# bwa-mem2/bwa-mem2

Hardware: NVIDIA H100
Metric: paired 151bp reads/s (seed+chain+extend hot path) (higher is better)
Workload: dtype int64/int16

## Files before the change

### bwa-mem2_b200/capi.py

```python
from __future__ import annotations
import ctypes as C, os
import numpy as np

_HERE = os.path.dirname(os.path.abspath(__file__))
LIB_PATH = os.path.join(_HERE, "libbm2b200.so")

PAIR_DT = np.dtype([("idr", "<i4"), ("idq", "<i4"), ("id", "<i4"), ("len1", "<i4"), ("len2", "<i4"), ("h0", "<i4"),
                    ("seqid", "<i4"), ("regid", "<i4"), ("score", "<i4"), ("tle", "<i4"), ("gtle", "<i4"),
                    ("qle", "<i4"), ("gscore", "<i4"), ("max_off", "<i4")])
SMEM_DT = np.dtype([("rid", "<u4"), ("m", "<u4"), ("n", "<u4"), ("_pad", "<u4"), ("k", "<i8"), ("l", "<i8"), ("s", "<i8")])
SEED_DT = np.dtype([("rbeg", "<i8"), ("qbeg", "<i4"), ("len", "<i4"), ("score", "<i4"), ("chain", "<i4")])
CHAIN_DT = np.dtype([("pos", "<i8"), ("seqid", "<i4"), ("rid", "<i4"), ("n_seeds", "<i4"), ("seed_off", "<i4"),
                     ("w", "<i4"), ("kept", "<i4"), ("first", "<i4"), ("is_alt", "<i4"), ("frac_rep", "<f4"), ("_pad", "<i4")])
REG_DT = np.dtype([("rb", "<i8"), ("re", "<i8"), ("qb", "<i4"), ("qe", "<i4"), ("rid", "<i4"), ("_p0", "<i4"), ("c", "<u8"),
                   ("score", "<i4"), ("truesc", "<i4"), ("sub", "<i4"), ("alt_sc", "<i4"), ("csub", "<i4"), ("sub_n", "<i4"),
                   ("w", "<i4"), ("seedcov", "<i4"), ("secondary", "<i4"), ("secondary_all", "<i4"), ("seedlen0", "<i4"),
                   ("n_comp_is_alt", "<i4"), ("frac_rep", "<f4"), ("_p1", "<i4"), ("hash", "<u8"), ("flg", "<i4"), ("_p2", "<i4")])


class MemOpt(C.Structure):
    _fields_ = [("a", C.c_int), ("b", C.c_int), ("o_del", C.c_int), ("e_del", C.c_int), ("o_ins", C.c_int), ("e_ins", C.c_int),
                ("pen_unpaired", C.c_int), ("pen_clip5", C.c_int), ("pen_clip3", C.c_int), ("w", C.c_int), ("zdrop", C.c_int),
                ("max_mem_intv", C.c_uint64), ("T", C.c_int), ("flag", C.c_int), ("min_seed_len", C.c_int),
                ("min_chain_weight", C.c_int), ("max_chain_extend", C.c_int), ("split_factor", C.c_float),
# ... 949 lines not shown

    def seed_chain_extend_resident(self, codes, offsets, d_codes_ptr, d_offsets_ptr, copy_out=False, return_arrays=False):
        rb, keep = self._batch(codes, offsets)
        res = RegResult()
        lib().bm2_seed_chain_extend_resident.argtypes = [C.c_void_p, C.c_void_p, C.c_void_p, C.c_void_p, C.c_int, C.c_void_p]
        self._check(lib().bm2_seed_chain_extend_resident(self._ctx, C.byref(rb), d_codes_ptr, d_offsets_ptr, int(copy_out), C.byref(res)),
                    "bm2_seed_chain_extend_resident")
        if not return_arrays:
            return res.n
        n = res.n
        regs = np.ctypeslib.as_array(C.cast(res.regs, C.POINTER(C.c_uint8)), shape=(n * REG_DT.itemsize,)).view(REG_DT).copy() if n else np.zeros(0, REG_DT)
        off = np.ctypeslib.as_array(C.cast(res.read_off, C.POINTER(C.c_int64)), shape=(rb.n_reads + 1,)).copy()
        return regs, off

    def counters(self):
        v = (C.c_ulonglong * 7)()
        lib().bm2_last_counters.argtypes = [C.c_void_p, C.c_void_p, C.c_int]
        lib().bm2_last_counters(self._ctx, v, 7)
        return dict(n_ext=v[0], n_lf=v[1], cells=v[2], retry_left=v[3], retry_right=v[4], jobs_skipped=v[5], reads_done_wave1=v[6])

    def stage_ms(self):
        names = C.POINTER(C.c_char_p)(); ms = C.POINTER(C.c_float)(); n = C.c_int()
        lib().bm2_last_stage_ms(self._ctx, C.byref(names), C.byref(ms), C.byref(n))
        return {names[i].decode(): ms[i] for i in range(n.value)}
```

### bwa-mem2_b200/csrc/bm2_ctx.h

```cpp
#pragma once
#include <cuda_runtime.h>
#include <string>
#include <type_traits>
#include <vector>
#include <mutex>
#include "bm2_b200.h"

struct DevBuf  { void *p = nullptr; size_t cap = 0; };
struct HostBuf { void *p = nullptr; size_t cap = 0; };

struct DevIndex {
    int64_t N = 0, l_pac = 0, sentinel = 0;
    int64_t count[5] = {0, 0, 0, 0, 0};
    const bm2_cp_occ *cp_occ = nullptr;
    int occ_layout = 0;
    const int8_t *sa_ms = nullptr;
    const uint32_t *sa_ls = nullptr;
    const uint8_t *ref = nullptr;
    int32_t n_seqs = 0;
    const int64_t *ann_off = nullptr;
    const int32_t *ann_len = nullptr;
    const int32_t *ann_alt = nullptr;
    bool loaded = false;
};

struct bm2_ctx {
    int device = 0, n_sm = 132;
    int fq_n_reads = 0, fq_n_bufs = 0;
    cudaStream_t stream = nullptr, own_stream = nullptr, side_stream = nullptr;
    cudaEvent_t ev_fork = nullptr, ev_join = nullptr;
    bm2_mem_opt_t opt;
    std::string err;
    DevIndex idx;
    std::vector<void *> idx_allocs;
    DevBuf io_pairs, io_ref, io_qer, bsw_jobs, bsw_outs, bsw_scratch;
    DevBuf pipe_d[39];
    HostBuf pipe_h[5];
    std::vector<cudaEvent_t> events;
    std::vector<const char *> stage_names;
    std::vector<float> stage_ms;
    unsigned long long last_n_ext = 0, last_n_lf = 0, last_cells = 0, last_n_retry[2] = {0, 0};
    unsigned long long last_jobs_skipped = 0, last_walk_done = 0;
    int n_lanes = 4, lane_min_reads = 16384;
    std::vector<bm2_ctx *> lanes;
    bm2_ctx *parent = nullptr;
    std::mutex tok_smem, tok_bsw;
    cudaEvent_t ev_entry = nullptr;
    DevBuf cigar_d[14];
    HostBuf cigar_h[3];
    DevBuf ksw_d[6];
    DevBuf fq_d[38];
    HostBuf fq_h[25];
    DevBuf sam_d[24];
    HostBuf sam_h[5];
    int sam_staged = -1;
    cudaEvent_t sam_ev[5] = {nullptr, nullptr, nullptr, nullptr, nullptr};
    double sam_ms[4] = {0, 0, 0, 0};
// ... 120 lines not shown
```

### bwa-mem2_b200/csrc/fm_device.cuh

```cuda
#pragma once
#include "hd.h"
#include "bm2_b200.h"

struct FmIndexView {
    const bm2_cp_occ *cp_occ;
    const int8_t *sa_ms;
    const uint32_t *sa_ls;
    int64_t count[5];
    int64_t sentinel;
    int layout = 0;
    const uint8_t *text = nullptr;
    int64_t text_len = 0;
};

#if defined(__CUDA_ARCH__)
BM2_D void fm_ld256(const void *p, uint64_t &a, uint64_t &b, uint64_t &c, uint64_t &d) {
    asm volatile("ld.global.nc.v2.u64 {%0,%1}, [%4];\n\t"
                 "ld.global.nc.v2.u64 {%2,%3}, [%4+16];" : "=l"(a), "=l"(b), "=l"(c), "=l"(d) : "l"(p));
}
#endif

struct FmIv { int64_t k, l, s; };

BM2_HD int64_t fm_count(const FmIndexView &fm, int a) {
    return a == 0 ? fm.count[0] : a == 1 ? fm.count[1] : a == 2 ? fm.count[2] : a == 3 ? fm.count[3] : fm.count[4];
}

// ... 62 lines not shown

BM2_HD int64_t fm_sa_of_row(const FmIndexView &fm, int64_t r, int *lf_steps, int64_t at_sentinel = 0) {
    int64_t steps = 0;
    while (r & 7) {
        const bm2_cp_occ *e = fm.cp_occ + (r >> 6);
        const int y = 63 - (int) (r & 63);
#if defined(__CUDA_ARCH__)
        const ulonglong2 *p = reinterpret_cast<const ulonglong2 *>(e);
        ulonglong2 c01 = __ldg(p), c23 = __ldg(p + 1), b01 = __ldg(p + 2), b23 = __ldg(p + 3);
        if (fm.layout) { const ulonglong2 t = c23; c23 = b01; b01 = t; }
        uint64_t cnt[4] = {c01.x, c01.y, c23.x, c23.y}, bits[4] = {b01.x, b01.y, b23.x, b23.y};
#else
        uint64_t cnt[4], bits[4];
        for (int b = 0; b < 4; ++b) { cnt[b] = (uint64_t) e->cp_count[b]; bits[b] = e->one_hot_bwt_str[b]; }
#endif
        int b = ((bits[0] >> y) & 1) ? 0 : ((bits[1] >> y) & 1) ? 1 : ((bits[2] >> y) & 1) ? 2 : ((bits[3] >> y) & 1) ? 3 : 4;
        if (b == 4) { if (lf_steps) *lf_steps += (int) steps; return at_sentinel; }
        const int yy = (int) (r & 63);
        const uint64_t mask = yy ? ~0ULL << (64 - yy) : 0ULL;
        uint64_t cb = b == 0 ? cnt[0] : b == 1 ? cnt[1] : b == 2 ? cnt[2] : cnt[3];
        uint64_t bb = b == 0 ? bits[0] : b == 1 ? bits[1] : b == 2 ? bits[2] : bits[3];
        r = fm_count(fm, b) + (int64_t) cb + BM2_POPC64(bb & mask);
        ++steps;
    }
    if (lf_steps) *lf_steps += (int) steps;
#if defined(__CUDA_ARCH__)
    int64_t sa = ((int64_t) __ldg(fm.sa_ms + (r >> 3)) << 32) + (int64_t) __ldg(fm.sa_ls + (r >> 3));
#else
    int64_t sa = ((int64_t) fm.sa_ms[r >> 3] << 32) + (int64_t) fm.sa_ls[r >> 3];
#endif
    return sa + steps;
}

BM2_HD int64_t fm_text_pos_of_row(const FmIndexView &fm, int64_t r) { return fm_sa_of_row(fm, r, nullptr, -1); }

struct FmPrev { int64_t k, l, s; int32_t m, n; };

struct SmemParams {
    int min_seed_len;
    int split_len;
    int split_width;
    int max_mem_intv;
};

struct QPlain {
    const uint8_t *p;
    BM2_HD int operator()(int j) const { return p[j]; }
};

// ... 56 lines not shown
                if (a > 3) { if (single) return; x = next_x; continue; }
                cur.m = x; cur.n = x; cur.k = fm_count(fm, a); cur.l = fm_count(fm, 3 - a); cur.s = fm_count(fm, a + 1) - cur.k;
                top = cap; j = x + 1; searching = true; tpos = -1;
            }
            bool stop = j >= len;
            if (!stop) { next_x = j + 1; const int a = q(j); if (a > 3) stop = true; else { base = 3 - a; need = true; } }
            if (stop) {
                if (cur.s >= min_intv) scratch[--top] = cur;
                sink(x, min_intv, scratch + top, cap - top);
                if (single) return;
                x = next_x; searching = false;
            }
        }
        BM2_SYNCWARP();
        FmIv r;
        if (fm.text && cur.s == 1 && tpos == -1) tpos = len - j >= 16 ? fm_text_pos_of_row(fm, cur.k) : -2;
        if (fm.text && cur.s == 1 && tpos >= 0) {
            const int64_t tp = tpos + (j - x);
            r.s = (tp < fm.text_len && (int) fm.text[tp] == 3 - base) ? 1 : 0;
            r.l = cur.k; r.k = cur.l;
        } else {
            if (tpos == -1 && fm.text && cur.s == 1) tpos = -2;
            FmIv req; req.k = cur.l; req.l = cur.k; req.s = cur.s;
            r = fm_backward_ext(fm, req, base);
        }
        ++n_ext;
        if (r.s != cur.s) scratch[--top] = cur;
        if (r.s < min_intv) {
            next_x = j;
            if (cur.s >= min_intv) scratch[--top] = cur;
            sink(x, min_intv, scratch + top, cap - top);
            if (single) return;
            x = next_x; searching = false;
        } else { cur.k = r.l; cur.l = r.k; cur.s = r.s; cur.n = j; ++j; }
    }
}

template <class Q, class Emit>
BM2_HD void fm_backward(const FmIndexView &fm, const Q &q, int x, int min_intv, int min_seed_len, FmPrev *pv, int num_prev, Emit &emit,
                        unsigned &n_ext)
{
    int j = x - 1, p = 0, num_curr = 0, curr_s = -1;
    bool first_phase = true;
    for (;;) {
        bool done = false;
        for (;;) {
            if (num_prev == 0 || j < 0) { done = true; break; }
            if (p == 0 && num_curr == 0 && first_phase && q(j) > 3) { done = true; break; }
            if (p < num_prev) break;
            num_prev = num_curr;
            if (num_curr == 0) { done = true; break; }
            --j; p = 0; num_curr = 0; curr_s = -1; first_phase = true;
        }
        if (done) break;
        BM2_SYNCWARP();
        const FmPrev old = pv[p];
        FmIv req; req.k = old.k; req.l = old.l; req.s = old.s;
        const FmIv r = fm_backward_ext(fm, req, q(j));
        ++n_ext;
        if (first_phase && r.s < min_intv && old.n - old.m + 1 >= min_seed_len) {
            emit(old.m, old.n, old.k, old.l, old.s);
            first_phase = false;
        } else if (r.s >= min_intv && r.s != curr_s) {
            curr_s = (int) r.s;
            FmPrev t; t.k = r.k; t.l = r.l; t.s = r.s; t.m = j; t.n = old.n;
            pv[num_curr++] = t;
            first_phase = false;
        }
        ++p;
    }
    if (num_prev != 0) {
        const FmPrev &s0 = pv[0];
        if (s0.n - s0.m + 1 >= min_seed_len) emit(s0.m, s0.n, s0.k, s0.l, s0.s);
    }
}

template <class Q, class Emit>
BM2_HD void fm_backward_rows(const FmIndexView &fm, const Q &q, int x, int min_intv, int min_seed_len, FmPrev *pv, int num_prev,
                             Emit &emit, unsigned &n_ext)
{
    for (int j = x - 1; j >= 0 && num_prev > 0; --j) {
        const int a = q(j);
        if (a > 3) break;
#ifdef BM2_TRACE_BWD_ROW
        BM2_TRACE_BWD_ROW(num_prev);
#endif
        int b = num_prev;
        const FmPrev first = pv[0];
        for (int p = 0; p < num_prev; ++p) {
            FmIv req; req.k = pv[p].k; req.l = pv[p].l; req.s = pv[p].s;
            const FmIv r = fm_backward_ext(fm, req, a);
            ++n_ext;
            pv[p].k = r.k; pv[p].l = r.l; pv[p].s = r.s;
            if (r.s >= min_intv && b == num_prev) b = p;
        }
        if (b > 0 && first.n - first.m + 1 >= min_seed_len) emit(first.m, first.n, first.k, first.l, first.s);
        int num_curr = 0;
        int64_t last_s = -1;
        for (int p = b; p < num_prev; ++p) {
            if (pv[p].s != last_s) { last_s = pv[p].s; FmPrev t = pv[p]; t.m = j; pv[num_curr++] = t; }
        }
        num_prev = num_curr;
    }
    if (num_prev != 0) {
        const FmPrev &s0 = pv[0];
        if (s0.n - s0.m + 1 >= min_seed_len) emit(s0.m, s0.n, s0.k, s0.l, s0.s);
    }
}
```

### bwa-mem2_b200/csrc/pipeline.cu

```cuda
#include "bm2_common.cuh"
#include "bm2_ctx.h"
#include "fm_device.cuh"
#include "chain_device.cuh"
#include "ext_device.cuh"
#include <cub/device/device_radix_sort.cuh>
#include <cub/device/device_scan.cuh>
#include <vector>
#include <algorithm>
#include <mutex>
#include <thread>
#include <string>
#include <cstring>
#include <cstdlib>
#include <cmath>

static_assert(sizeof(ExtJobRec) == sizeof(BswJob), "ExtJobRec must alias BswJob");

int bsw_launch_with_scratch(bm2_ctx *ctx_for_error, cudaStream_t stream, const BswJob *d_jobs, BswOut *d_out, int n,
                            const uint8_t *d_tbase, const uint8_t *d_qbase, const BswParams &prm,
                            unsigned long long *d_cells, void *scratch, size_t scratch_bytes, int wide_possible);

__global__ void occ_relayout_kernel(ulonglong2 *tab, size_t n_entries) {
    const size_t i = (size_t) blockIdx.x * blockDim.x + threadIdx.x;
    if (i >= n_entries) return;
    ulonglong2 *e = tab + i * 4;
    const ulonglong2 c23 = e[1], b01 = e[2];
    e[1] = b01; e[2] = c23;
}

int bm2_upload_index(bm2_ctx *ctx, const bm2_index_desc *idx, int resident) {
    bm2_ctx *ctx_for_error = ctx;
    auto up = [&](const void *src, size_t bytes, const void **dst, bool big) -> int {
        if (big && resident) { *dst = src; return 0; }
        void *p = nullptr;
        BM2_CUDA_OK(cudaMalloc(&p, bytes ? bytes : 1));
        ctx->idx_allocs.push_back(p);
        if (bytes) BM2_CUDA_OK(cudaMemcpy(p, src, bytes, cudaMemcpyHostToDevice));
        *dst = p;
        return 0;
    };
    DevIndex &d = ctx->idx;
    d.N = idx->reference_seq_len; d.l_pac = idx->l_pac; d.sentinel = idx->sentinel_index;
// ... 1 lines not shown
    d.n_seqs = idx->n_seqs;
    size_t n_occ = (size_t) (d.N >> 6) + 1, n_sa = (size_t) (d.N >> 3) + 1;
    if (up(idx->cp_occ, n_occ * sizeof(bm2_cp_occ), (const void **) &d.cp_occ, true)) return 1;
    {
        const char *e = getenv("BM2_OCC_LAYOUT");
        d.occ_layout = (e && e[0] == '0') ? 0 : 1;
        if (d.occ_layout) {
            occ_relayout_kernel<<<(unsigned) ((n_occ + 255) / 256), 256>>>((ulonglong2 *) d.cp_occ, n_occ);
            BM2_CUDA_OK(cudaGetLastError());
            BM2_CUDA_OK(cudaDeviceSynchronize());
        }
    }
    if (up(idx->sa_ms_byte, n_sa, (const void **) &d.sa_ms, true)) return 1;
    if (up(idx->sa_ls_word, n_sa * 4, (const void **) &d.sa_ls, true)) return 1;
    if (up(idx->ref_string, (size_t) d.l_pac * 2, (const void **) &d.ref, true)) return 1;
    if (up(idx->ann_offset, (size_t) d.n_seqs * 8, (const void **) &d.ann_off, false)) return 1;
    if (up(idx->ann_len, (size_t) d.n_seqs * 4, (const void **) &d.ann_len, false)) return 1;
    std::vector<int32_t> zeros;
    const int32_t *alt = idx->ann_is_alt;
    if (!alt) { zeros.assign(d.n_seqs, 0); alt = zeros.data(); }
    if (up(alt, (size_t) d.n_seqs * 4, (const void **) &d.ann_alt, false)) return 1;
    d.loaded = true;
    return 0;
}

void bm2_free_index(bm2_ctx *ctx) {
    for (void *p : ctx->idx_allocs) cudaFree(p);
    ctx->idx_allocs.clear();
    ctx->idx.loaded = false;
}

struct Counters {
    unsigned long long n_smem, n_ext, n_lf, n_retry, cells;
    unsigned long long n_pool, n_task, n_task1, n_rtask;
    unsigned long long n_sel[2], n_walk_done;
};

struct SearchTask { int32_t read, x, min_intv, n; int64_t off; };
struct ReseedTask { int32_t read, x, min_intv; };


struct QShared4 {
    unsigned base, stride;
    __device__ __forceinline__ int operator()(int j) const {
        uint32_t w; asm volatile("ld.shared.u32 %0, [%1];" : "=r"(w) : "r"(base + (unsigned) (j >> 3) * stride));
        return (int) ((w >> ((j & 7) * 4)) & 0xFu);
    }
};

struct PoolSink {
// ... 70 lines not shown
        if (rtasks && n + 1 - m >= split_len && s <= split_width) {
            unsigned long long t = atomicAdd(&cnt->n_rtask, 1ULL);
            if (t < rtask_cap) { ReseedTask r; r.read = (int32_t) rid; r.x = (n + 1 + m) >> 1; r.min_intv = (int32_t) (s + 1); rtasks[t] = r; }
        }
    }
};

#define BWD_G 8
#define BWD_CAP 32
__global__ void __launch_bounds__(128, 8)
smem_bwd_kernel(FmIndexView fm, SmemParams sp, const uint8_t *__restrict__ codes, const int64_t *__restrict__ offs, int round,
                const SearchTask *__restrict__ tasks, unsigned long long task_cap, FmPrev *pool, unsigned long long pool_cap,
                bm2_smem *out, unsigned long long cap, ReseedTask *rtasks, unsigned long long rtask_cap, Counters *cnt)
{
    __shared__ FmPrev shl[128 / BWD_G][BWD_CAP];
    const int lane = threadIdx.x & 31, gl = lane & (BWD_G - 1), gw = lane / BWD_G;
    const unsigned gmask = ((1u << BWD_G) - 1u) << (gw * BWD_G);
    const int grp = (blockIdx.x * blockDim.x + threadIdx.x) / BWD_G, ngrp = gridDim.x * blockDim.x / BWD_G;
    const unsigned long long t0 = round ? cnt->n_task1 : 0ULL;
    const unsigned long long t1 = cnt->n_task < task_cap ? cnt->n_task : task_cap;
    unsigned n_ext = 0;
    for (unsigned long long t = t0 + grp; t < t1; t += ngrp) {
        const SearchTask k = tasks[t];
        if ((unsigned long long) k.off + k.n > pool_cap) continue;
        SmemAppend emit = { out, cap, cnt, (uint32_t) k.read, round ? nullptr : rtasks, rtask_cap, sp.split_len, sp.split_width };
        const uint8_t *q = codes + offs[k.read];
        FmPrev *lst = pool + k.off;
        int num_prev = k.n;
        if (num_prev <= BWD_CAP) {
            FmPrev *sl = shl[threadIdx.x / BWD_G];
            for (int p = gl; p < num_prev; p += BWD_G) sl[p] = lst[p];
            lst = sl;
        }
        __syncwarp(gmask);
        for (int j = k.x - 1; j >= 0 && num_prev > 0; --j) {
            const int a = q[j];
            if (a > 3) break;
            const FmPrev first = lst[0];
            __syncwarp(gmask);
            int b = num_prev;
            for (int p = gl; p < num_prev; p += BWD_G) {
                FmIv req; req.k = lst[p].k; req.l = lst[p].l; req.s = lst[p].s;
                const FmIv r = fm_backward_ext(fm, req, a);
                ++n_ext;
                lst[p].k = r.k; lst[p].l = r.l; lst[p].s = r.s;
                if (r.s >= k.min_intv && p < b) b = p;
            }
#pragma unroll
            for (int d = BWD_G / 2; d > 0; d >>= 1) b = min(b, __shfl_xor_sync(gmask, b, d));
            __syncwarp(gmask);
            if (gl == 0 && b > 0 && first.n - first.m + 1 >= sp.min_seed_len) emit(first.m, first.n, first.k, first.l, first.s);
            int num_curr = 0;
            for (int base = b; base < num_prev; base += BWD_G) {
                const int p = base + gl;
                bool keep = false;
                FmPrev e;
                if (p < num_prev) { e = lst[p]; keep = (p == b) || (lst[p - 1].s != e.s); }
                const unsigned km = __ballot_sync(gmask, keep) >> (gw * BWD_G);
                __syncwarp(gmask);
                if (keep) { e.m = j; lst[num_curr + __popc(km & ((1u << gl) - 1u))] = e; }
                num_curr += __popc(km);
                __syncwarp(gmask);
            }
            num_prev = num_curr;
        }
        if (gl == 0 && num_prev != 0) {
            const FmPrev s0 = lst[0];
            if (s0.n - s0.m + 1 >= sp.min_seed_len) emit(s0.m, s0.n, s0.k, s0.l, s0.s);
        }
        __syncwarp(gmask);
    }
    n_ext = __reduce_add_sync(0xffffffffu, n_ext);
    if (lane == 0 && n_ext) atomicAdd(&cnt->n_ext, (unsigned long long) n_ext);
}

__global__ void mark_task1_kernel(Counters *cnt) { if (threadIdx.x == 0 && blockIdx.x == 0) cnt->n_task1 = cnt->n_task; }

template <bool USE_SMEM>
__global__ void __launch_bounds__(128, 12)
smem_pass3_kernel(FmIndexView fm, SmemParams sp, const uint8_t *__restrict__ codes, const int64_t *__restrict__ offs, int n_reads,
                  bm2_smem *out, unsigned long long cap, Counters *cnt)
{
    extern __shared__ uint32_t qsh[];
    const int tid = blockIdx.x * blockDim.x + threadIdx.x, nthr = gridDim.x * blockDim.x;
    unsigned n_ext = 0;
    for (int r = tid; r < n_reads; r += nthr) {
        const int64_t o = offs[r];
        const int len = (int) (offs[r + 1] - o);
// ... 5 lines not shown
        } else {
            QPlain q = { codes + o };
            fm_smem_pass3(fm, q, len, sp, emit, n_ext);
        }
    }
    if (n_ext) atomicAdd(&cnt->n_ext, (unsigned long long) n_ext);
}

__global__ void smem_keys_kernel(const bm2_smem *sm, int64_t n, uint64_t *keys, uint32_t *vals) {
    int64_t i = (int64_t) blockIdx.x * blockDim.x + threadIdx.x;
    if (i >= n) return;
    keys[i] = (uint64_t) sm[i].rid << 32 | (uint64_t) (sm[i].m & 0xFFFFu) << 16 | (uint64_t) (sm[i].n & 0xFFFFu);
    vals[i] = (uint32_t) i;
}

__global__ void smem_gather_kernel(const bm2_smem *in, const uint32_t *perm, int64_t n, int max_occ, bm2_smem *out, int64_t *slot_cnt) {
    int64_t i = (int64_t) blockIdx.x * blockDim.x + threadIdx.x;
    if (i >= n) return;
    bm2_smem x = in[perm[i]];
    out[i] = x;
    slot_cnt[i] = x.s < max_occ ? x.s : max_occ;
}

__global__ void read_smem_off_kernel(const uint64_t *keys_sorted, int64_t n_smem, int n_reads, int64_t *read_smem_off) {
    int r = blockIdx.x * blockDim.x + threadIdx.x;
    if (r > n_reads) return;
    const uint64_t key = (uint64_t) r << 32;
    int64_t lo = 0, hi = n_smem;
    while (lo < hi) { int64_t mid = (lo + hi) >> 1; if (keys_sorted[mid] < key) lo = mid + 1; else hi = mid; }
    read_smem_off[r] = lo;
}

__global__ void slot_head_kernel(const int64_t *__restrict__ slot_off, int64_t n_smem, int32_t *owner) {
    int64_t i = (int64_t) blockIdx.x * blockDim.x + threadIdx.x;
    if (i >= n_smem) return;
    if (slot_off[i + 1] > slot_off[i]) owner[slot_off[i]] = (int32_t) i;
}

__global__ void __launch_bounds__(256)
sa_kernel(FmIndexView fm, const bm2_smem *__restrict__ sm, const int64_t *__restrict__ slot_off, const int32_t *__restrict__ owner,
          int64_t n_slots, int max_occ, int64_t *sa, Counters *cnt)
{
    int64_t t = (int64_t) blockIdx.x * blockDim.x + threadIdx.x;
    int lf = 0;
    if (t < n_slots) {
        const int32_t o = owner[t];
        const bm2_smem x = sm[o];
        const int64_t step = x.s > max_occ ? x.s / max_occ : 1;
        sa[t] = fm_sa_of_row(fm, x.k + (t - slot_off[o]) * step, &lf);
    }
    lf = __reduce_add_sync(0xffffffffu, lf);
    if ((threadIdx.x & 31) == 0 && lf) atomicAdd(&cnt->n_lf, (unsigned long long) lf);
}

struct ChainBufs {
    WSeed *wseed; WChain *wchain; int32_t *ord, *srt, *kv; int64_t *ordpos; FltRec *flt;
    bm2_chain *fin_chain; bm2_seed *fin_seed;
    int32_t *n_chain, *n_seed, *n_left, *n_right;
};

__global__ void __launch_bounds__(128)
chain_kernel(ContigView cv, ChainParams cp, const bm2_smem *__restrict__ sm, const int64_t *__restrict__ read_smem_off,
             const int64_t *__restrict__ slot_off, const int64_t *__restrict__ sa, const int64_t *__restrict__ offs, int n_reads,
             const int32_t *__restrict__ perm, ChainBufs b, SwParams sw, const uint8_t *__restrict__ ref, const uint8_t *__restrict__ codes,
// ... 529 lines not shown
        for (int r = 0; r < n; ++r) {
            const int64_t l = rb->offsets[r + 1] - rb->offsets[r];
            if (l < 0 || l > 32767) { bm2_set_error(ctx, "read length out of range (0..32767)"); return 1; }
            if (l > max_len) max_len = (int) l;
            if (l != memo_l) {
                const double min_l = ctx->opt.min_chain_weight ? 1.1f * ctx->opt.min_chain_weight : 5.5f * log((double) (l > 0 ? l : 1));
                memo_l = l; memo_hsp = -1;
                if (l > 0 && !(min_l > 0.05f * l)) memo_hsp = (int) (ctx->opt.a * min_l + .499);
            }
            if (memo_hsp >= 0 && !any_flt) { any_flt = true; min_hsp_host.assign((size_t) n, -1); }
            if (any_flt) min_hsp_host[r] = memo_hsp;
        }
    }
    bs.max_len = max_len;
    Params pv = make_params(ctx);
    if (upto != UPTO_SMEM && env_int("BM2_SMEM_TEXT", 1, 0, 1)) { pv.fm.text = ctx->idx.ref; pv.fm.text_len = 2 * ctx->idx.l_pac; }
    Stages sg = { ctx, ctx->events, ctx->stage_names };
    if (sg.mark("h2d")) return 1;

    if (ctx->ensure(ctx->pipe_d[B_CNT], sizeof(Counters))) return 1;
    const uint8_t *d_codes = ext_codes; const int64_t *d_offs = ext_offs;
    if (!ext_codes) {
        if (ctx->ensure(ctx->pipe_d[B_CODES], (size_t) total + 16)) return 1;
        BM2_CUDA_OK(cudaMemcpyAsync(ctx->pipe_d[B_CODES].p, rb->codes, (size_t) total, cudaMemcpyHostToDevice, st));
        d_codes = P<uint8_t>(ctx, B_CODES);
    }
    if (!ext_offs) {
        if (ctx->ensure(ctx->pipe_d[B_OFFS], (size_t) (n + 1) * 8)) return 1;
        BM2_CUDA_OK(cudaMemcpyAsync(ctx->pipe_d[B_OFFS].p, rb->offsets, (size_t) (n + 1) * 8, cudaMemcpyHostToDevice, st));
        d_offs = P<int64_t>(ctx, B_OFFS);
    }
// ... 49 lines not shown
        smem_fwd2_kernel<<<blocks_a, 128, 0, st>>>(pv.fm, d_codes, d_offs, stripe, P<FmPrev>(ctx, B_PREV), d_rt, rtask_cap, d_pool, pool_cap, d_tasks, task_cap, d_cnt);
        smem_bwd_kernel<<<blocks_b, 128, 0, st>>>(pv.fm, pv.sp, d_codes, d_offs, 1, d_tasks, task_cap, d_pool, pool_cap, d_raw, cap, d_rt, rtask_cap, d_cnt);
        BM2_CUDA_OK(cudaStreamWaitEvent(st, ctx->ev_join, 0));
        BM2_CUDA_OK(cudaMemcpyAsync(&h_cnt, d_cnt, sizeof(Counters), cudaMemcpyDeviceToHost, st));
        BM2_CUDA_OK(cudaStreamSynchronize(st));
        if (h_cnt.n_smem <= cap && h_cnt.n_pool <= pool_cap && h_cnt.n_task <= task_cap && h_cnt.n_rtask <= rtask_cap) break;
        if (attempt == 2) { bm2_set_error(ctx, "SMEM stage buffers overflow"); return 1; }
        if (h_cnt.n_smem > cap) cap = h_cnt.n_smem * 2 + 1024;
        if (h_cnt.n_pool > pool_cap) pool_cap = h_cnt.n_pool * 2 + 65536;
        if (h_cnt.n_task > task_cap) task_cap = h_cnt.n_task * 2 + 4096;
        if (h_cnt.n_rtask > rtask_cap) rtask_cap = h_cnt.n_rtask * 2 + 4096;
    }
    tok_smem.release();
    const int64_t n_smem = (int64_t) h_cnt.n_smem;
    bs.n_smem = n_smem;
    ctx->last_n_ext = h_cnt.n_ext;

    if (sg.mark("sort")) return 1;
    const int64_t ns1 = n_smem > 0 ? n_smem : 1;
    if (ctx->ensure(ctx->pipe_d[B_KEYS_IN], ns1 * 8) || ctx->ensure(ctx->pipe_d[B_KEYS_OUT], ns1 * 8) || ctx->ensure(ctx->pipe_d[B_VALS_IN], ns1 * 4) ||
        ctx->ensure(ctx->pipe_d[B_VALS_OUT], ns1 * 4) || ctx->ensure(ctx->pipe_d[B_SMEM], (ns1 + 1) * sizeof(bm2_smem)) ||
        ctx->ensure(ctx->pipe_d[B_SLOT_CNT], (ns1 + 1) * 8) || ctx->ensure(ctx->pipe_d[B_SLOT_OFF], (ns1 + 2) * 8) ||
        ctx->ensure(ctx->pipe_d[B_READ_SMEM_OFF], (size_t) (n + 2) * 8)) return 1;
    if (n_smem > 0) {
        const int gb = (int) ((n_smem + 255) / 256);
        smem_keys_kernel<<<gb, 256, 0, st>>>(P<bm2_smem>(ctx, B_SMEM_RAW), n_smem, P<uint64_t>(ctx, B_KEYS_IN), P<uint32_t>(ctx, B_VALS_IN));
        size_t cub_bytes = 0;
        cub::DeviceRadixSort::SortPairs(nullptr, cub_bytes, P<uint64_t>(ctx, B_KEYS_IN), P<uint64_t>(ctx, B_KEYS_OUT), P<uint32_t>(ctx, B_VALS_IN),
                                        P<uint32_t>(ctx, B_VALS_OUT), (int) n_smem);
        if (ctx->ensure(ctx->pipe_d[B_CUB], cub_bytes)) return 1;
        BM2_CUDA_OK(cub::DeviceRadixSort::SortPairs(ctx->pipe_d[B_CUB].p, cub_bytes, P<uint64_t>(ctx, B_KEYS_IN), P<uint64_t>(ctx, B_KEYS_OUT),
                                                    P<uint32_t>(ctx, B_VALS_IN), P<uint32_t>(ctx, B_VALS_OUT), (int) n_smem, 0, 64, st));
        BM2_CUDA_OK(cudaMemsetAsync(P<int64_t>(ctx, B_SLOT_CNT) + n_smem, 0, 8, st));
        smem_gather_kernel<<<gb, 256, 0, st>>>(P<bm2_smem>(ctx, B_SMEM_RAW), P<uint32_t>(ctx, B_VALS_OUT), n_smem, ctx->opt.max_occ,
                                               P<bm2_smem>(ctx, B_SMEM), P<int64_t>(ctx, B_SLOT_CNT));
    } else {
        BM2_CUDA_OK(cudaMemsetAsync(P<int64_t>(ctx, B_SLOT_CNT), 0, 8, st));
    }
    read_smem_off_kernel<<<(n + 1 + 255) / 256, 256, 0, st>>>(P<uint64_t>(ctx, B_KEYS_OUT), n_smem, n, P<int64_t>(ctx, B_READ_SMEM_OFF));
    if (scan64(ctx, P<int64_t>(ctx, B_SLOT_CNT), P<int64_t>(ctx, B_SLOT_OFF), n_smem)) return 1;
    if (upto == UPTO_SMEM) { if (sg.mark("end")) return 1; BM2_CUDA_OK(cudaStreamSynchronize(st)); return 0; }
    int64_t n_slots = 0;
    BM2_CUDA_OK(cudaMemcpyAsync(&n_slots, P<int64_t>(ctx, B_SLOT_OFF) + n_smem, 8, cudaMemcpyDeviceToHost, st));
    BM2_CUDA_OK(cudaStreamSynchronize(st));
    bs.n_slots = n_slots;
    if (n_slots > (int64_t) 1500000000) { bm2_set_error(ctx, "too many seed occurrences in one batch: use smaller chunks"); return 1; }

    if (sg.mark("sal")) return 1;
    const size_t sl1 = (size_t) (n_slots > 0 ? n_slots : 1) + 1;
    if (ctx->ensure(ctx->pipe_d[B_SA], sl1 * 8)) return 1;
// ... 46 lines not shown
    char *scb = (char *) ctx->pipe_d[B_SCAN].p;
    int64_t *w_tmp = (int64_t *) scb, *d_chain_off = (int64_t *) (scb + sc), *d_reg_off = (int64_t *) (scb + 2 * sc),
            *d_left_off = (int64_t *) (scb + 3 * sc), *d_right_off = (int64_t *) (scb + 4 * sc), *d_out_off = (int64_t *) (scb + 5 * sc);
    const int gw = (n + 1 + 255) / 256;
    widen_kernel<<<gw, 256, 0, st>>>(d_nchain, n, w_tmp); if (scan64(ctx, w_tmp, d_chain_off, n)) return 1;
    widen_kernel<<<gw, 256, 0, st>>>(d_nseed, n, w_tmp);  if (scan64(ctx, w_tmp, d_reg_off, n)) return 1;
    widen_kernel<<<gw, 256, 0, st>>>(d_nleft, n, w_tmp);  if (scan64(ctx, w_tmp, d_left_off, n)) return 1;
    widen_kernel<<<gw, 256, 0, st>>>(d_nright, n, w_tmp); if (scan64(ctx, w_tmp, d_right_off, n)) return 1;
    int64_t tot[4];
    BM2_CUDA_OK(cudaMemcpyAsync(&tot[0], d_chain_off + n, 8, cudaMemcpyDeviceToHost, st));
    BM2_CUDA_OK(cudaMemcpyAsync(&tot[1], d_reg_off + n, 8, cudaMemcpyDeviceToHost, st));
    BM2_CUDA_OK(cudaMemcpyAsync(&tot[2], d_left_off + n, 8, cudaMemcpyDeviceToHost, st));
    BM2_CUDA_OK(cudaMemcpyAsync(&tot[3], d_right_off + n, 8, cudaMemcpyDeviceToHost, st));
    BM2_CUDA_OK(cudaMemcpyAsync(&h_cnt, d_cnt, sizeof(Counters), cudaMemcpyDeviceToHost, st));
    BM2_CUDA_OK(cudaStreamSynchronize(st));
    ctx->last_n_lf = h_cnt.n_lf;
    const int64_t n_chains = tot[0], n_regs = tot[1], n_left = tot[2], n_right = tot[3];
    bs.n_chains = n_chains; bs.n_regs = n_regs; bs.n_left = n_left; bs.n_right = n_right;
    if (n_regs > 2000000000LL) { bm2_set_error(ctx, "too many seeds in one batch"); return 1; }
    if (ctx->ensure(ctx->pipe_d[B_CHAINS], (size_t) (n_chains + 1) * sizeof(bm2_chain)) || ctx->ensure(ctx->pipe_d[B_SEEDS], (size_t) (n_regs + 1) * sizeof(bm2_seed))) return 1;
    chain_compact_kernel<<<(n + 127) / 128, 128, 0, st>>>(P<int64_t>(ctx, B_READ_SMEM_OFF), P<int64_t>(ctx, B_SLOT_OFF), n, P<bm2_chain>(ctx, B_FIN_CHAIN),
                                                          P<bm2_seed>(ctx, B_FIN_SEED), d_chain_off, d_reg_off, P<bm2_chain>(ctx, B_CHAINS), P<bm2_seed>(ctx, B_SEEDS));
    if (upto == UPTO_CHAIN) { if (sg.mark("end")) return 1; BM2_CUDA_OK(cudaStreamSynchronize(st)); return 0; }

    if (sg.mark("extbuild")) return 1;
    const size_t nr1 = (size_t) n_regs + 1, nl1 = (size_t) n_left + 1, nrt1 = (size_t) n_right + 1;
    const int lazy = env_int("BM2_EXT_LAZY", 1, 0, 1);
    const int waves = env_int("BM2_EXT_WAVES", 2, 2, 64);
    const size_t aux_bytes = al(nr1 * 4) * 3 + al(nr1 * 8) + al(nl1 * 4) * 2 + al(nrt1 * 4) * 2 + al(nr1 * sizeof(PfBox)) +
                             (lazy ? al(nr1) + al((size_t) n * sizeof(PfCursor)) + al(nl1 * 4) + al(nrt1 * 4) : 0);
    const size_t njmax = nl1 > nrt1 ? nl1 : nrt1;
// ... 266 lines not shown
    int64_t pos = 0;
    for (int k = 0; k < K; ++k) {
        const Job &j = jobs[k];
        bm2_ctx *l = ctx->lanes[k];
        const int64_t *lo = (const int64_t *) l->pipe_h[H_OUT_OFF].p;
        if (copy_out && j.bs.n_out)
            BM2_CUDA_OK(cudaMemcpyAsync(regs + pos, l->pipe_d[B_OUT].p, (size_t) j.bs.n_out * sizeof(bm2_alnreg_t), cudaMemcpyDeviceToHost, l->stream));
        for (int i = 0; i < j.n; ++i) off[j.first + i] = lo[i] + pos;
        pos += j.bs.n_out;
    }
    off[n] = n_out;
    for (int k = 0; k < K; ++k) BM2_CUDA_OK(cudaStreamSynchronize(ctx->lanes[k]->stream));
    ctx->stage_names = ctx->lanes[0]->stage_names;
    ctx->stage_ms.assign(ctx->lanes[0]->stage_ms.size(), 0.f);
    ctx->last_n_ext = ctx->last_n_lf = ctx->last_cells = 0; ctx->last_n_retry[0] = ctx->last_n_retry[1] = 0;
    ctx->last_jobs_skipped = ctx->last_walk_done = 0;
    for (int k = 0; k < K; ++k) {
        const bm2_ctx *l = ctx->lanes[k];
        for (size_t i = 0; i < ctx->stage_ms.size() && i < l->stage_ms.size(); ++i) ctx->stage_ms[i] += l->stage_ms[i];
        ctx->last_n_ext += l->last_n_ext; ctx->last_n_lf += l->last_n_lf; ctx->last_cells += l->last_cells;
        ctx->last_n_retry[0] += l->last_n_retry[0]; ctx->last_n_retry[1] += l->last_n_retry[1];
        ctx->last_jobs_skipped += l->last_jobs_skipped; ctx->last_walk_done += l->last_walk_done;
    }
    out->n = n_out; out->regs = copy_out ? regs : nullptr; out->read_off = off;
    return 0;
}

extern "C" int bm2_seed_chain_extend(bm2_ctx *ctx, const bm2_read_batch *reads, bm2_reg_result *out) {
    if (!ctx || !reads || !out) return 1;
    return run_regs(ctx, reads, nullptr, nullptr, true, out);
}

extern "C" int bm2_seed_chain_extend_resident(bm2_ctx *ctx, const bm2_read_batch *reads, const uint8_t *d_codes, const int64_t *d_offsets,
                                              int copy_out, bm2_reg_result *out) {
    if (!ctx || !reads || !out || !d_codes || !d_offsets) return 1;
    return run_regs(ctx, reads, d_codes, d_offsets, copy_out != 0, out);
}

extern "C" int bm2_last_stage_ms(const bm2_ctx *ctx, const char *const **names, const float **ms, int *n) {
    if (!ctx) return 1;
    *names = ctx->stage_names.data(); *ms = ctx->stage_ms.data();
    *n = (int) (ctx->stage_ms.size() < ctx->stage_names.size() ? ctx->stage_ms.size() : ctx->stage_names.size());
    return 0;
}

extern "C" int bm2_last_counters(const bm2_ctx *ctx, unsigned long long *v, int n) {
    if (!ctx || n < 5) return 1;
    v[0] = ctx->last_n_ext; v[1] = ctx->last_n_lf; v[2] = ctx->last_cells; v[3] = ctx->last_n_retry[0]; v[4] = ctx->last_n_retry[1];
    if (n >= 7) { v[5] = ctx->last_jobs_skipped; v[6] = ctx->last_walk_done; }
    return 0;
}
```

Before: 10.28 million.

## Carry singleton SMEM intervals as text positions to skip FM and SA lookups

```diff
diff --git a/bwa-mem2_b200/capi.py b/bwa-mem2_b200/capi.py
--- a/bwa-mem2_b200/capi.py
+++ b/bwa-mem2_b200/capi.py
@@ -987,10 +987,11 @@
         return regs, off
 
     def counters(self):
-        v = (C.c_ulonglong * 7)()
+        v = (C.c_ulonglong * 9)()
         lib().bm2_last_counters.argtypes = [C.c_void_p, C.c_void_p, C.c_int]
-        lib().bm2_last_counters(self._ctx, v, 7)
-        return dict(n_ext=v[0], n_lf=v[1], cells=v[2], retry_left=v[3], retry_right=v[4], jobs_skipped=v[5], reads_done_wave1=v[6])
+        lib().bm2_last_counters(self._ctx, v, 9)
+        return dict(n_ext=v[0], n_lf=v[1], cells=v[2], retry_left=v[3], retry_right=v[4], jobs_skipped=v[5], reads_done_wave1=v[6],
+                    n_text_ext=v[7], n_sa_carried=v[8])
 
     def stage_ms(self):
         names = C.POINTER(C.c_char_p)(); ms = C.POINTER(C.c_float)(); n = C.c_int()
diff --git a/bwa-mem2_b200/csrc/bm2_ctx.h b/bwa-mem2_b200/csrc/bm2_ctx.h
--- a/bwa-mem2_b200/csrc/bm2_ctx.h
+++ b/bwa-mem2_b200/csrc/bm2_ctx.h
@@ -17,6 +17,7 @@
     const int8_t *sa_ms = nullptr;
     const uint32_t *sa_ls = nullptr;
     const uint8_t *ref = nullptr;
+    int64_t sa_p0 = 0;
     int32_t n_seqs = 0;
     const int64_t *ann_off = nullptr;
     const int32_t *ann_len = nullptr;
@@ -41,6 +42,7 @@
     std::vector<float> stage_ms;
     unsigned long long last_n_ext = 0, last_n_lf = 0, last_cells = 0, last_n_retry[2] = {0, 0};
     unsigned long long last_jobs_skipped = 0, last_walk_done = 0;
+    unsigned long long last_n_text = 0, last_n_sa_carried = 0;
     int n_lanes = 4, lane_min_reads = 16384;
     std::vector<bm2_ctx *> lanes;
     bm2_ctx *parent = nullptr;
diff --git a/bwa-mem2_b200/csrc/fm_device.cuh b/bwa-mem2_b200/csrc/fm_device.cuh
--- a/bwa-mem2_b200/csrc/fm_device.cuh
+++ b/bwa-mem2_b200/csrc/fm_device.cuh
@@ -11,6 +11,8 @@
     int layout = 0;
     const uint8_t *text = nullptr;
     int64_t text_len = 0;
+    int carry = 0;
+    int64_t sa_p0 = 0;
 };
 
 #if defined(__CUDA_ARCH__)
@@ -103,6 +105,9 @@
         uint64_t cnt[4], bits[4];
         for (int b = 0; b < 4; ++b) { cnt[b] = (uint64_t) e->cp_count[b]; bits[b] = e->one_hot_bwt_str[b]; }
 #endif
+#if defined(BM2_TRACE_LF) && !defined(__CUDA_ARCH__)
+        BM2_TRACE_LF(r);
+#endif
         int b = ((bits[0] >> y) & 1) ? 0 : ((bits[1] >> y) & 1) ? 1 : ((bits[2] >> y) & 1) ? 2 : ((bits[3] >> y) & 1) ? 3 : 4;
         if (b == 4) { if (lf_steps) *lf_steps += (int) steps; return at_sentinel; }
         const int yy = (int) (r & 63);
@@ -117,11 +122,48 @@
     int64_t sa = ((int64_t) __ldg(fm.sa_ms + (r >> 3)) << 32) + (int64_t) __ldg(fm.sa_ls + (r >> 3));
 #else
     int64_t sa = ((int64_t) fm.sa_ms[r >> 3] << 32) + (int64_t) fm.sa_ls[r >> 3];
+#if defined(BM2_TRACE_SA)
+    BM2_TRACE_SA(r);
+#endif
 #endif
     return sa + steps;
 }
 
 BM2_HD int64_t fm_text_pos_of_row(const FmIndexView &fm, int64_t r) { return fm_sa_of_row(fm, r, nullptr, -1); }
+
+BM2_HD int64_t fm_sa_of_smem_row(const FmIndexView &fm, int64_t k, int *lf_steps) {
+    if (k < 0) { const int64_t tp = -1 - k; return tp >= fm.sa_p0 ? tp : 0; }
+    return fm_sa_of_row(fm, k, lf_steps);
+}
+
+template <class E>
+BM2_HD int64_t fm_backward_step(const FmIndexView &fm, E &e, int a, unsigned *n_text) {
+    const int64_t k = e.k;
+    int t = 4;
+#if defined(__CUDA_ARCH__)
+    if (k < -1) {
+        unsigned v;
+        asm volatile("ld.global.nc.u8 %0, [%1];" : "=r"(v) : "l"(fm.text - 2 - k));
+        t = (int) v;
+    }
+#else
+    if (k < -1) t = fm.text[-2 - k];
+#if defined(BM2_TRACE_TEXT)
+    if (k < -1) BM2_TRACE_TEXT(-2 - k);
+#endif
+#endif
+    if (k >= 0) {
+        FmIv req; req.k = k; req.l = e.l; req.s = e.s;
+        const FmIv r = fm_backward_ext(fm, req, a);
+        e.k = r.k; e.l = r.l; e.s = r.s;
+        return r.s;
+    }
+    const int s1 = t == a;
+    e.k = k + s1;
+    e.s = s1;
+    if (n_text) ++*n_text;
+    return s1;
+}
 
 struct FmPrev { int64_t k, l, s; int32_t m, n; };
 
@@ -208,10 +250,16 @@
         }
         BM2_SYNCWARP();
         FmIv r;
-        if (fm.text && cur.s == 1 && tpos == -1) tpos = len - j >= 16 ? fm_text_pos_of_row(fm, cur.k) : -2;
+        if (fm.text && cur.s == 1 && tpos == -1) {
+            tpos = len - j >= 16 ? fm_text_pos_of_row(fm, cur.k) : -2;
+            if (fm.carry && tpos >= 0) cur.k = -1 - tpos;
+        }
         if (fm.text && cur.s == 1 && tpos >= 0) {
             const int64_t tp = tpos + (j - x);
             r.s = (tp < fm.text_len && (int) fm.text[tp] == 3 - base) ? 1 : 0;
+#if defined(BM2_TRACE_TEXT) && !defined(__CUDA_ARCH__)
+            BM2_TRACE_TEXT(tp);
+#endif
             r.l = cur.k; r.k = cur.l;
         } else {
             if (tpos == -1 && fm.text && cur.s == 1) tpos = -2;
@@ -232,7 +280,7 @@
 
 template <class Q, class Emit>
 BM2_HD void fm_backward(const FmIndexView &fm, const Q &q, int x, int min_intv, int min_seed_len, FmPrev *pv, int num_prev, Emit &emit,
-                        unsigned &n_ext)
+                        unsigned &n_ext, unsigned *n_text = nullptr)
 {
     int j = x - 1, p = 0, num_curr = 0, curr_s = -1;
     bool first_phase = true;
@@ -249,8 +297,8 @@
         if (done) break;
         BM2_SYNCWARP();
         const FmPrev old = pv[p];
-        FmIv req; req.k = old.k; req.l = old.l; req.s = old.s;
-        const FmIv r = fm_backward_ext(fm, req, q(j));
+        FmIv r; r.k = old.k; r.l = old.l; r.s = old.s;
+        fm_backward_step(fm, r, q(j), n_text);
         ++n_ext;
         if (first_phase && r.s < min_intv && old.n - old.m + 1 >= min_seed_len) {
             emit(old.m, old.n, old.k, old.l, old.s);
@@ -271,7 +319,7 @@
 
 template <class Q, class Emit>
 BM2_HD void fm_backward_rows(const FmIndexView &fm, const Q &q, int x, int min_intv, int min_seed_len, FmPrev *pv, int num_prev,
-                             Emit &emit, unsigned &n_ext)
+                             Emit &emit, unsigned &n_ext, unsigned *n_text = nullptr)
 {
     for (int j = x - 1; j >= 0 && num_prev > 0; --j) {
         const int a = q(j);
@@ -282,11 +330,9 @@
         int b = num_prev;
         const FmPrev first = pv[0];
         for (int p = 0; p < num_prev; ++p) {
-            FmIv req; req.k = pv[p].k; req.l = pv[p].l; req.s = pv[p].s;
-            const FmIv r = fm_backward_ext(fm, req, a);
+            const int64_t s1 = fm_backward_step(fm, pv[p], a, n_text);
             ++n_ext;
-            pv[p].k = r.k; pv[p].l = r.l; pv[p].s = r.s;
-            if (r.s >= min_intv && b == num_prev) b = p;
+            if (s1 >= min_intv && b == num_prev) b = p;
         }
         if (b > 0 && first.n - first.m + 1 >= min_seed_len) emit(first.m, first.n, first.k, first.l, first.s);
         int num_curr = 0;
diff --git a/bwa-mem2_b200/csrc/pipeline.cu b/bwa-mem2_b200/csrc/pipeline.cu
--- a/bwa-mem2_b200/csrc/pipeline.cu
+++ b/bwa-mem2_b200/csrc/pipeline.cu
@@ -26,6 +26,17 @@
     ulonglong2 *e = tab + i * 4;
     const ulonglong2 c23 = e[1], b01 = e[2];
     e[1] = b01; e[2] = c23;
+}
+
+__global__ void sa_min_kernel(const int8_t *ms, const uint32_t *ls, size_t n, unsigned long long *out) {
+    unsigned long long m = ~0ULL;
+    for (size_t i = (size_t) blockIdx.x * blockDim.x + threadIdx.x; i < n; i += (size_t) gridDim.x * blockDim.x) {
+        const unsigned long long v = (unsigned long long) (((int64_t) ms[i] << 32) + (int64_t) ls[i]);
+        m = v < m ? v : m;
+    }
+#pragma unroll
+    for (int d = 16; d > 0; d >>= 1) { const unsigned long long o = __shfl_xor_sync(0xffffffffu, m, d); m = o < m ? o : m; }
+    if ((threadIdx.x & 31) == 0 && m != ~0ULL) atomicMin(out, m);
 }
 
 int bm2_upload_index(bm2_ctx *ctx, const bm2_index_desc *idx, int resident) {
@@ -57,6 +68,18 @@
     if (up(idx->sa_ms_byte, n_sa, (const void **) &d.sa_ms, true)) return 1;
     if (up(idx->sa_ls_word, n_sa * 4, (const void **) &d.sa_ls, true)) return 1;
     if (up(idx->ref_string, (size_t) d.l_pac * 2, (const void **) &d.ref, true)) return 1;
+    {
+        unsigned long long *d_min = nullptr, h_min = ~0ULL;
+        BM2_CUDA_OK(cudaMalloc(&d_min, 8));
+        BM2_CUDA_OK(cudaMemcpy(d_min, &h_min, 8, cudaMemcpyHostToDevice));
+        const size_t n_samp = (size_t) ((d.N + 7) >> 3);
+        sa_min_kernel<<<(unsigned) std::min<size_t>((n_samp + 255) / 256, 8192), 256>>>(d.sa_ms, d.sa_ls, n_samp, d_min);
+        BM2_CUDA_OK(cudaGetLastError());
+        const cudaError_t e = cudaMemcpy(&h_min, d_min, 8, cudaMemcpyDeviceToHost);
+        cudaFree(d_min);
+        BM2_CUDA_OK(e);
+        d.sa_p0 = h_min == ~0ULL ? 0 : (int64_t) h_min;
+    }
     if (up(idx->ann_offset, (size_t) d.n_seqs * 8, (const void **) &d.ann_off, false)) return 1;
     if (up(idx->ann_len, (size_t) d.n_seqs * 4, (const void **) &d.ann_len, false)) return 1;
     std::vector<int32_t> zeros;
@@ -77,6 +100,7 @@
     unsigned long long n_smem, n_ext, n_lf, n_retry, cells;
     unsigned long long n_pool, n_task, n_task1, n_rtask;
     unsigned long long n_sel[2], n_walk_done;
+    unsigned long long n_text, n_sa_carried;
 };
 
 struct SearchTask { int32_t read, x, min_intv, n; int64_t off; };
@@ -177,12 +201,13 @@
                 bm2_smem *out, unsigned long long cap, ReseedTask *rtasks, unsigned long long rtask_cap, Counters *cnt)
 {
     __shared__ FmPrev shl[128 / BWD_G][BWD_CAP];
+    __shared__ FmPrev shfirst[128 / BWD_G];
     const int lane = threadIdx.x & 31, gl = lane & (BWD_G - 1), gw = lane / BWD_G;
     const unsigned gmask = ((1u << BWD_G) - 1u) << (gw * BWD_G);
     const int grp = (blockIdx.x * blockDim.x + threadIdx.x) / BWD_G, ngrp = gridDim.x * blockDim.x / BWD_G;
     const unsigned long long t0 = round ? cnt->n_task1 : 0ULL;
     const unsigned long long t1 = cnt->n_task < task_cap ? cnt->n_task : task_cap;
-    unsigned n_ext = 0;
+    unsigned n_ext = 0, n_text = 0;
     for (unsigned long long t = t0 + grp; t < t1; t += ngrp) {
         const SearchTask k = tasks[t];
         if ((unsigned long long) k.off + k.n > pool_cap) continue;
@@ -199,20 +224,20 @@
         for (int j = k.x - 1; j >= 0 && num_prev > 0; --j) {
             const int a = q[j];
             if (a > 3) break;
-            const FmPrev first = lst[0];
-            __syncwarp(gmask);
+            if (gl == 0) shfirst[threadIdx.x / BWD_G] = lst[0];
             int b = num_prev;
             for (int p = gl; p < num_prev; p += BWD_G) {
-                FmIv req; req.k = lst[p].k; req.l = lst[p].l; req.s = lst[p].s;
-                const FmIv r = fm_backward_ext(fm, req, a);
+                const int64_t s1 = fm_backward_step(fm, lst[p], a, &n_text);
                 ++n_ext;
-                lst[p].k = r.k; lst[p].l = r.l; lst[p].s = r.s;
-                if (r.s >= k.min_intv && p < b) b = p;
+                if (s1 >= k.min_intv && p < b) b = p;
             }
 #pragma unroll
             for (int d = BWD_G / 2; d > 0; d >>= 1) b = min(b, __shfl_xor_sync(gmask, b, d));
             __syncwarp(gmask);
-            if (gl == 0 && b > 0 && first.n - first.m + 1 >= sp.min_seed_len) emit(first.m, first.n, first.k, first.l, first.s);
+            if (gl == 0 && b > 0) {
+                const FmPrev first = shfirst[threadIdx.x / BWD_G];
+                if (first.n - first.m + 1 >= sp.min_seed_len) emit(first.m, first.n, first.k, first.l, first.s);
+            }
             int num_curr = 0;
             for (int base = b; base < num_prev; base += BWD_G) {
                 const int p = base + gl;
@@ -234,7 +259,9 @@
         __syncwarp(gmask);
     }
     n_ext = __reduce_add_sync(0xffffffffu, n_ext);
+    n_text = __reduce_add_sync(0xffffffffu, n_text);
     if (lane == 0 && n_ext) atomicAdd(&cnt->n_ext, (unsigned long long) n_ext);
+    if (lane == 0 && n_text) atomicAdd(&cnt->n_text, (unsigned long long) n_text);
 }
 
 __global__ void mark_task1_kernel(Counters *cnt) { if (threadIdx.x == 0 && blockIdx.x == 0) cnt->n_task1 = cnt->n_task; }
@@ -270,12 +297,18 @@
     vals[i] = (uint32_t) i;
 }
 
-__global__ void smem_gather_kernel(const bm2_smem *in, const uint32_t *perm, int64_t n, int max_occ, bm2_smem *out, int64_t *slot_cnt) {
+__global__ void smem_gather_kernel(const bm2_smem *in, const uint32_t *perm, int64_t n, int max_occ, bm2_smem *out, int64_t *slot_cnt,
+                                   Counters *cnt) {
     int64_t i = (int64_t) blockIdx.x * blockDim.x + threadIdx.x;
-    if (i >= n) return;
-    bm2_smem x = in[perm[i]];
-    out[i] = x;
-    slot_cnt[i] = x.s < max_occ ? x.s : max_occ;
+    int carried = 0;
+    if (i < n) {
+        bm2_smem x = in[perm[i]];
+        out[i] = x;
+        slot_cnt[i] = x.s < max_occ ? x.s : max_occ;
+        carried = x.k < 0;
+    }
+    carried = __reduce_add_sync(0xffffffffu, carried);
+    if ((threadIdx.x & 31) == 0 && carried) atomicAdd(&cnt->n_sa_carried, (unsigned long long) carried);
 }
 
 __global__ void read_smem_off_kernel(const uint64_t *keys_sorted, int64_t n_smem, int n_reads, int64_t *read_smem_off) {
@@ -303,7 +336,7 @@
         const int32_t o = owner[t];
         const bm2_smem x = sm[o];
         const int64_t step = x.s > max_occ ? x.s / max_occ : 1;
-        sa[t] = fm_sa_of_row(fm, x.k + (t - slot_off[o]) * step, &lf);
+        sa[t] = fm_sa_of_smem_row(fm, x.k + (t - slot_off[o]) * step, &lf);
     }
     lf = __reduce_add_sync(0xffffffffu, lf);
     if ((threadIdx.x & 31) == 0 && lf) atomicAdd(&cnt->n_lf, (unsigned long long) lf);
@@ -863,7 +896,10 @@
     }
     bs.max_len = max_len;
     Params pv = make_params(ctx);
-    if (upto != UPTO_SMEM && env_int("BM2_SMEM_TEXT", 1, 0, 1)) { pv.fm.text = ctx->idx.ref; pv.fm.text_len = 2 * ctx->idx.l_pac; }
+    if (upto != UPTO_SMEM && env_int("BM2_SMEM_TEXT", 1, 0, 1)) {
+        pv.fm.text = ctx->idx.ref; pv.fm.text_len = 2 * ctx->idx.l_pac;
+        pv.fm.carry = env_int("BM2_SMEM_CARRY", 1, 0, 1); pv.fm.sa_p0 = ctx->idx.sa_p0;
+    }
     Stages sg = { ctx, ctx->events, ctx->stage_names };
     if (sg.mark("h2d")) return 1;
 
@@ -943,7 +979,7 @@
     tok_smem.release();
     const int64_t n_smem = (int64_t) h_cnt.n_smem;
     bs.n_smem = n_smem;
-    ctx->last_n_ext = h_cnt.n_ext;
+    ctx->last_n_ext = h_cnt.n_ext; ctx->last_n_text = h_cnt.n_text;
 
     if (sg.mark("sort")) return 1;
     const int64_t ns1 = n_smem > 0 ? n_smem : 1;
@@ -962,7 +998,7 @@
                                                     P<uint32_t>(ctx, B_VALS_IN), P<uint32_t>(ctx, B_VALS_OUT), (int) n_smem, 0, 64, st));
         BM2_CUDA_OK(cudaMemsetAsync(P<int64_t>(ctx, B_SLOT_CNT) + n_smem, 0, 8, st));
         smem_gather_kernel<<<gb, 256, 0, st>>>(P<bm2_smem>(ctx, B_SMEM_RAW), P<uint32_t>(ctx, B_VALS_OUT), n_smem, ctx->opt.max_occ,
-                                               P<bm2_smem>(ctx, B_SMEM), P<int64_t>(ctx, B_SLOT_CNT));
+                                               P<bm2_smem>(ctx, B_SMEM), P<int64_t>(ctx, B_SLOT_CNT), d_cnt);
     } else {
         BM2_CUDA_OK(cudaMemsetAsync(P<int64_t>(ctx, B_SLOT_CNT), 0, 8, st));
     }
@@ -1039,7 +1075,7 @@
     BM2_CUDA_OK(cudaMemcpyAsync(&tot[3], d_right_off + n, 8, cudaMemcpyDeviceToHost, st));
     BM2_CUDA_OK(cudaMemcpyAsync(&h_cnt, d_cnt, sizeof(Counters), cudaMemcpyDeviceToHost, st));
     BM2_CUDA_OK(cudaStreamSynchronize(st));
-    ctx->last_n_lf = h_cnt.n_lf;
+    ctx->last_n_lf = h_cnt.n_lf; ctx->last_n_sa_carried = h_cnt.n_sa_carried;
     const int64_t n_chains = tot[0], n_regs = tot[1], n_left = tot[2], n_right = tot[3];
     bs.n_chains = n_chains; bs.n_regs = n_regs; bs.n_left = n_left; bs.n_right = n_right;
     if (n_regs > 2000000000LL) { bm2_set_error(ctx, "too many seeds in one batch"); return 1; }
@@ -1336,13 +1372,14 @@
     ctx->stage_names = ctx->lanes[0]->stage_names;
     ctx->stage_ms.assign(ctx->lanes[0]->stage_ms.size(), 0.f);
     ctx->last_n_ext = ctx->last_n_lf = ctx->last_cells = 0; ctx->last_n_retry[0] = ctx->last_n_retry[1] = 0;
-    ctx->last_jobs_skipped = ctx->last_walk_done = 0;
+    ctx->last_jobs_skipped = ctx->last_walk_done = 0; ctx->last_n_text = ctx->last_n_sa_carried = 0;
     for (int k = 0; k < K; ++k) {
         const bm2_ctx *l = ctx->lanes[k];
         for (size_t i = 0; i < ctx->stage_ms.size() && i < l->stage_ms.size(); ++i) ctx->stage_ms[i] += l->stage_ms[i];
         ctx->last_n_ext += l->last_n_ext; ctx->last_n_lf += l->last_n_lf; ctx->last_cells += l->last_cells;
         ctx->last_n_retry[0] += l->last_n_retry[0]; ctx->last_n_retry[1] += l->last_n_retry[1];
         ctx->last_jobs_skipped += l->last_jobs_skipped; ctx->last_walk_done += l->last_walk_done;
+        ctx->last_n_text += l->last_n_text; ctx->last_n_sa_carried += l->last_n_sa_carried;
     }
     out->n = n_out; out->regs = copy_out ? regs : nullptr; out->read_off = off;
     return 0;
@@ -1370,5 +1407,6 @@
     if (!ctx || n < 5) return 1;
     v[0] = ctx->last_n_ext; v[1] = ctx->last_n_lf; v[2] = ctx->last_cells; v[3] = ctx->last_n_retry[0]; v[4] = ctx->last_n_retry[1];
     if (n >= 7) { v[5] = ctx->last_jobs_skipped; v[6] = ctx->last_walk_done; }
+    if (n >= 9) { v[7] = ctx->last_n_text; v[8] = ctx->last_n_sa_carried; }
     return 0;
 }
```

Result: no change. 10.28 million (median of 6 runs) (+0.0%).
